# danielbrathwaite/OpenGL-Path-Tracing

Measured on AMD Instinct MI355X. Metric: Mrays/sec + ms/frame @1920×1080, 8 bounces, 1/2/4/8 MI355X, higher is better.
Workload: dtype f32; 1 GPU; C2: cornell 1920x1080, 1024 spp (frames 1..1024), 8 bounces (i<=8), AA+sky+sphere on; scene=cornell, width=1920, height=1080, spp=1024, max_bounce=8, frames_per_launch=1024, kernel_variant=0, parallelism=single GPU

## Files before the change

### opengl-path-tracing_amd/csrc/pt_cull.h

```cpp
#pragma once

#include "pt_math.h"

namespace ptc {

constexpr float kWindowLo = 0.0001f * 0x1.ff8p-1f;
constexpr float kWindowRay = 0x1.4p-20f;

PT_HD float min_t(float tf, float t) {
#if defined(__HIP_DEVICE_COMPILE__)
    return __builtin_amdgcn_fmed3f(tf, t, -__builtin_huge_valf());
#else
    return fminf(tf, t);
#endif
}

PT_HD void cull_addends(pt::f3 o, pt::f3 rd, const float cm[3], const float ws[3], pt::f3& ol, pt::f3& oh) {
    const pt::f3 ord = pt::mk(-(o.x * rd.x), -(o.y * rd.y), -(o.z * rd.z));
    const float ax = __builtin_fabsf(rd.x), ay = __builtin_fabsf(rd.y), az = __builtin_fabsf(rd.z);
    const pt::f3 e = pt::mk(__builtin_fmaf(cm[0], ax, 0x1p-17f * __builtin_fabsf(ord.x)),
                            __builtin_fmaf(cm[1], ay, 0x1p-17f * __builtin_fabsf(ord.y)),
                            __builtin_fmaf(cm[2], az, 0x1p-17f * __builtin_fabsf(ord.z)));
    const float omax = fmaxf(fmaxf(__builtin_fabsf(o.x), __builtin_fabsf(o.y)), __builtin_fabsf(o.z));
    const float wx = __builtin_fmaf(kWindowRay, omax, ws[0]), wy = __builtin_fmaf(kWindowRay, omax, ws[1]),
                wz = __builtin_fmaf(kWindowRay, omax, ws[2]);
    ol = ord - e;
    oh = ord + pt::mk(__builtin_fmaf(wx, ax, e.x), __builtin_fmaf(wy, ay, e.y), __builtin_fmaf(wz, az, e.z));
}

PT_HD bool cull_hit(float nx, float fx, float ny, float fy, float nz, float fz, pt::f3 rd, pt::f3 ol, pt::f3 oh,
                    float cur_t, float c_lo) {
    const float xn = __builtin_fmaf(nx, rd.x, ol.x), xf = __builtin_fmaf(fx, rd.x, oh.x);
    const float yn = __builtin_fmaf(ny, rd.y, ol.y), yf = __builtin_fmaf(fy, rd.y, oh.y);
    const float zn = __builtin_fmaf(nz, rd.z, ol.z), zf = __builtin_fmaf(fz, rd.z, oh.z);
    const float tn = fmaxf(fmaxf(xn, yn), zn);
    const float tf = fminf(fminf(xf, yf), zf);
    return fmaxf(tn, c_lo) <= min_t(tf, cur_t);
}

inline bool window_slack(const float* bvh, int n_nodes, const float* tris, float ws[3]) {
    const double u = 0x1p-24;
    const float inf = __builtin_huge_valf();
    ws[0] = ws[1] = ws[2] = 0.0f;
    if (n_nodes <= 0) return true;
    double M2 = 0.0;
    for (int q = 0; q < 3; q++) {
        const double m = fmax(fabs((double)bvh[q]), fabs((double)bvh[4 + q]));
        M2 += m * m;
    }
    M2 = sqrt(M2);
    double worst[3] = {0.0, 0.0, 0.0};
    for (int i = 0; i < n_nodes; i++) {
        const float* nd = bvh + 12 * (size_t)i;
        if (!(nd[8] > -1.0f)) continue;
        for (int k = 0; k < 2; k++) {
            const float* t = tris + 16 * (size_t)(int)nd[8 + k];
            const pt::f3 v0 = pt::mk(t[0], t[1], t[2]), v1 = pt::mk(t[4], t[5], t[6]), v2 = pt::mk(t[8], t[9], t[10]);
            const pt::f3 n = pt::normalize(pt::cross(v1 - v0, v2 - v0));
            const float d0 = -pt::dot(n, v0);
            if (!(fabs((double)n.x) + fabs((double)n.y) + fabs((double)n.z) < (double)inf)) continue;
            const double V[3][3] = {{v0.x, v0.y, v0.z}, {v1.x, v1.y, v1.z}, {v2.x, v2.y, v2.z}};
            const double nn[3] = {n.x, n.y, n.z};
            double E1[3], E2[3], L2 = 0.0, rho = 0.0;
            for (int q = 0; q < 3; q++) { E1[q] = V[1][q] - V[0][q]; E2[q] = V[2][q] - V[0][q]; }
            const double N[3] = {E1[1] * E2[2] - E2[1] * E1[2], E1[2] * E2[0] - E2[2] * E1[0], E1[0] * E2[1] - E2[0] * E1[1]};
            const double D = nn[0] * N[0] + nn[1] * N[1] + nn[2] * N[2];
            for (int a = 0; a < 3; a++) {
                const int b = (a + 1) % 3;
                double l2 = 0.0;
                for (int q = 0; q < 3; q++) l2 += (V[b][q] - V[a][q]) * (V[b][q] - V[a][q]);
                L2 = fmax(L2, l2);
                rho = fmax(rho, fabs(nn[0] * V[a][0] + nn[1] * V[a][1] + nn[2] * V[a][2] + (double)d0));
            }
            const double L = sqrt(L2);
            if (!(D > 0.0) || !(L2 <= 0x1p14 * D) || !(rho <= L)) return false;
            const double kappa = L2 / D, z = 1.06 * 0x1p-140 * L / D;
            const double sigma_t = u * (7.2 * M2 + 4.4 * fabs((double)d0)) + 1.14 * rho + 6.5 * z;
            for (int q = 0; q < 3; q++) {
                const double ext = fmax(fmax(V[0][q], V[1][q]), V[2][q]) - fmin(fmin(V[0][q], V[1][q]), V[2][q]);
                worst[q] = fmax(worst[q], 21.4 * u * kappa * ext + 1.021 * sigma_t + 2.0 * z);
            }
        }
    }
    for (int q = 0; q < 3; q++)
        if (!(worst[q] < 0x1p60)) return false;
    for (int q = 0; q < 3; q++) ws[q] = nextafterf((float)(1.25 * worst[q] * (1.0 + 0x1p-20)), inf);
    return true;
}

struct SweepRay { pt::f3 rp, rn, ol, oh; };
PT_HD SweepRay sweep_ray(pt::f3 rd, pt::f3 ol, pt::f3 oh) {
    SweepRay r;
    r.rp = pt::mk(rd.x > 0.0f ? rd.x : 0.0f, rd.y > 0.0f ? rd.y : 0.0f, rd.z > 0.0f ? rd.z : 0.0f);
    r.rn = pt::mk(rd.x > 0.0f ? 0.0f : rd.x, rd.y > 0.0f ? 0.0f : rd.y, rd.z > 0.0f ? 0.0f : rd.z);
    r.ol = ol;
    r.oh = oh;
    return r;
}
PT_HD bool sweep_hit(float lx, float hx, float ly, float hy, float lz, float hz, const SweepRay& r, float t0, float c_lo) {
    const float xn = __builtin_fmaf(lx, r.rp.x, __builtin_fmaf(hx, r.rn.x, r.ol.x));
    const float xf = __builtin_fmaf(hx, r.rp.x, __builtin_fmaf(lx, r.rn.x, r.oh.x));
    const float yn = __builtin_fmaf(ly, r.rp.y, __builtin_fmaf(hy, r.rn.y, r.ol.y));
    const float yf = __builtin_fmaf(hy, r.rp.y, __builtin_fmaf(ly, r.rn.y, r.oh.y));
    const float zn = __builtin_fmaf(lz, r.rp.z, __builtin_fmaf(hz, r.rn.z, r.ol.z));
    const float zf = __builtin_fmaf(hz, r.rp.z, __builtin_fmaf(lz, r.rn.z, r.oh.z));
    const float tn = fmaxf(fmaxf(xn, yn), zn);
    const float tf = fminf(fminf(xf, yf), zf);
    return fmaxf(tn, c_lo) <= min_t(tf, t0);
}
PT_HD unsigned sweep_push(unsigned m, bool hit) {
#if defined(__HIP_DEVICE_COMPILE__) && !defined(PT_SWEEP_NO_ADDC)
    unsigned r;
    const unsigned long long c = __builtin_amdgcn_ballot_w64(hit);
    unsigned long long co;
    asm("v_addc_co_u32 %0, %1, %2, %2, %3" : "=v"(r), "=s"(co) : "v"(m), "s"(c));
    return r;
#else
    return m + m + (hit ? 1u : 0u);
#endif
}
template <class T>
PT_HD unsigned sweep_mask(const SweepRay& r, float t0, float c_lo, T table, int n) {
    unsigned m = 0u;
    for (int k = n - 1; k >= 0; k--) {
        const auto a = table[2 * k], b = table[2 * k + 1];
        m = sweep_push(m, sweep_hit(a.x, a.y, a.z, a.w, b.x, b.y, r, t0, c_lo));
    }
    return m;
}
template <class T>
PT_HD unsigned sweep_mask(pt::f3 rd, pt::f3 ol, pt::f3 oh, float t0, float c_lo, T table, int n) {
    return sweep_mask(sweep_ray(rd, ol, oh), t0, c_lo, table, n);
}
PT_HD bool sweep_root_hit(const float box[6], const SweepRay& r, float t0, float c_lo) {
    return sweep_hit(box[0], box[1], box[2], box[3], box[4], box[5], r, t0, c_lo);
}

}
```

### opengl-path-tracing_amd/csrc/pt_render_phase.h

```cpp
namespace {

typedef float v4f __attribute__((ext_vector_type(4)));
typedef __attribute__((address_space(3))) const v4f lds_v4f;
typedef __attribute__((address_space(4))) const v4f const_v4f;

template <bool LDS>
__device__ __forceinline__ float4 tri_quad(const SceneView& S, int slot, int k) {
#ifdef PT_DIAG_TRIS_GLOBAL
    return S.tris[4 * slot + k];
#else
    return LDS ? S.tris[slot + k * S.tp] : S.tris[4 * slot + k];
#endif
}

using pt::in_guard;
using pt::in_range_abs;

using pt::win_open;
using pt::win_closed;

__device__ __forceinline__ int rank_in(unsigned long long m) {
    return (int)__builtin_amdgcn_mbcnt_hi((unsigned)(m >> 32), __builtin_amdgcn_mbcnt_lo((unsigned)m, 0u));
}

template <bool COMMON, bool SWEEP = false>
struct LaunchFacts {
    const KParams& p;
    __device__ __forceinline__ bool sweep() const { return COMMON ? SWEEP : p.sweep != 0; }
    __device__ __forceinline__ int mode() const { return COMMON ? 1 : p.mode; }
    __device__ __forceinline__ int flags() const { return COMMON ? 0 : p.flags; }
    __device__ __forceinline__ bool cons_walk() const { return COMMON || p.cons_walk != 0; }
    __device__ __forceinline__ bool scene_fast() const { return COMMON || p.scene_fast != 0; }
    __device__ __forceinline__ float win_lo() const { return COMMON ? ptc::kWindowLo : p.win_lo; }
    __device__ __forceinline__ int n_spheres() const { return COMMON ? 1 : p.sc.n_spheres; }
    __device__ __forceinline__ int tile_shift() const { return COMMON ? 0 : p.tile_shift; }
    __device__ __forceinline__ bool tile_perm() const { return COMMON || p.tile_perm != nullptr; }
    __device__ __forceinline__ bool tile_cost() const { return COMMON || p.tile_cost != nullptr; }
    __device__ __forceinline__ bool inside(int cx, int cy) const { return COMMON || ((cx < p.x_limit) & (cy < p.y_limit)); }
};

__device__ __forceinline__ void stage_tris_chain_order(float4* dst, const KParams& p, int T, int nthreads) {
    for (int i = threadIdx.x; i < 4 * T; i += nthreads) {
        const int slot = i >> 2, c = __float_as_int(p.sweep_tab[2 * (slot >> 1) + 1].w);
        dst[(i & 3) * T + 2 * c + (slot & 1)] = p.sc.tris[i];
    }
}

template <bool LDS, class Facts>
__device__ __forceinline__ bool shade_segment(const Facts& F, const KParams& p, const SceneView& S, bool hit, int hprim,
                                              float t, f3& o, f3& d, f3& inc, f3& col, uint32_t& state, int& bounce,
                                              f3& rgb) {
    bool finished = false;
    rgb = inc;
    if (hit && pt::length_gt_001(col)) {
        const f3 hitp = o + d * t;
        f3 normal;
        int mat;
        if (hprim >= 0) {
            const float4 nq = tri_quad<LDS>(S, hprim, 0);
            normal = mk(nq.x, nq.y, nq.z);
            mat = __float_as_int(tri_quad<LDS>(S, hprim, 2).w);
        } else {
            const int si = -2 - hprim;
            float4 s0 = S.spheres[2 * si];
            normal = pt::normalize(hitp - mk(s0.x, s0.y, s0.z));
            mat = __float_as_int(S.spheres[2 * si + 1].x);
        }
        if (pt::dot(normal, d) > 0.0f) normal = normal * -1.0f;
        if (F.mode() == 2) {
            rgb = (normal + mk(1, 1, 1)) * 0.5f;
            finished = true;
        } else if (F.mode() == 4) {
            float s = pt::length(hitp - o);
            float dist = 1.0f - pt::fsqrt(s + 1.0f) / (s + 1.0f);
            float q = dist * dist;
            rgb = mk(q, q, q);
            finished = true;
        } else {
            o = hitp;
            f3 diffuse = pt::normalize(normal + pt::random_unit_vector(state));
            float kk = 2.0f * pt::dot(normal, d);
            f3 specular = pt::normalize(d - normal * kk);
            float4 m0 = S.mats[3 * mat], m1 = S.mats[3 * mat + 1], m2 = S.mats[3 * mat + 2];
            if (F.mode() == 3) {
                rgb = mk(m0.x, m0.y, m0.z);
                finished = true;
            } else {
                float is_spec = (m1.w > pt::random01(state)) ? 1.0f : 0.0f;
                d = pt::mix(diffuse, specular, m0.w * is_spec);
                inc = inc + mk(m1.x, m1.y, m1.z) * col;
                col = col * pt::mix(mk(m0.x, m0.y, m0.z), mk(m2.x, m2.y, m2.z), is_spec);
                bounce++;
                if (bounce > p.max_bounce) {
                    rgb = inc;
                    finished = true;
                }
            }
        }
    } else {
        f3 env = mk(0, 0, 0);
        if (!(F.flags() & PT_FLAG_NO_SKY)) {
            f3 dir = pt::normalize(d);
            float tt = 0.5f * (dir.z + 1.0f);
            float omt = 1.0f - tt;
            env = mk(omt * 1.0f + tt * 0.5f, omt * 1.0f + tt * 0.7f, omt * 1.0f + tt * 1.0f);
        }
        rgb = inc + env * col;
        finished = true;
    }
    return finished;
}

struct QueueIds { unsigned id, qnext, qend; };
template <bool SPLIT>
__device__ __forceinline__ QueueIds queue_ids(const KParams& p, bool want, unsigned long long m, unsigned qnext,
                                              unsigned qend) {
    const unsigned need = (unsigned)__popcll(m);
    const unsigned rank = (unsigned)rank_in(m);
    const int leader = __ffsll((long long)m) - 1;
    unsigned id;
    if (SPLIT && qend - qnext >= need) {
        id = qnext + rank;
        qnext += need;
    } else {
        const unsigned avail = SPLIT ? qend - qnext : 0u;
        const unsigned take = SPLIT ? max(need - avail, (unsigned)p.pull_batch) : need;
        unsigned base = 0;
        if (want && rank == 0u) base = atomicAdd(p.work_counter, take);
        base = (unsigned)__builtin_amdgcn_readlane((int)base, leader);
        id = rank < avail ? qnext + rank : base + (rank - avail);
        if (SPLIT) {
            qnext = base + (need - avail);
            qend = base + take;
        }
    }
    const QueueIds q = {id, qnext, qend};
    return q;
}

template <class Facts>
__device__ __forceinline__ void camera_ray(const Facts& F, const KParams& p, f3 cpos, f3 cfwd, f3 cright, f3 cup, int lx,
                                           int y, int k, int r, uint32_t& state, f3& o, f3& d, f3& inc, f3& col,
                                           int& bounce) {
    if (r == 0) state = pt::seed(lx, y, p.frame_first + k);
    float ax = 0.0f, ay = 0.0f;
    if (!(F.flags() & PT_FLAG_NO_AA)) {
        ax = pt::random01(state);
        ay = pt::random01(state);
    }
    float u = pt::div_mk((float)lx + ax, p.fW, p.rW) - 0.5f;
    float v = pt::div_mk((float)y + ay, p.fH, p.rH) - 0.5f;
    d = pt::normalize((cfwd + cright * u) + cup * v);
    o = cpos;
    inc = mk(0, 0, 0);
    col = mk(1, 1, 1);
    bounce = 0;
}

template <class Facts>
__device__ __forceinline__ bool seg_in_guard(const Facts& F, f3 o, f3 d) {
    return F.scene_fast() & in_guard(o.x, 0x1p-40f, 0x1p60f) & in_guard(o.y, 0x1p-40f, 0x1p60f) &
           in_guard(o.z, 0x1p-40f, 0x1p60f) & in_range_abs(d.x, 0x1p-20f, 2.0f) &
           in_range_abs(d.y, 0x1p-20f, 2.0f) & in_range_abs(d.z, 0x1p-20f, 2.0f);
}

__device__ __forceinline__ float sphere_t(const SceneView& S, int si, f3 o, f3 d) {
    float4 s0 = S.spheres[2 * si];
    f3 oc = o - mk(s0.x, s0.y, s0.z);
    float a = pt::dot(d, d);
    float half_b = pt::dot(oc, d);
    float cq = pt::dot(oc, oc) - s0.w;
    float disc = half_b * half_b - a * cq;
    return disc < 0.0f ? -1.0f : (-half_b - pt::sqrt_g(disc)) / a;
}

__device__ __forceinline__ unsigned sweep_candidates(const KParams& p, const SceneView& S, const const_v4f* sweep_tab,
                                                     bool on, f3 o, f3 rd, float t) {
    unsigned cand = 0u;
    if (on) {
        f3 ol, oh;
        ptc::cull_addends(o, rd, S.cm, S.ws, ol, oh);
        const ptc::SweepRay sr = ptc::sweep_ray(rd, ol, oh);
        bool in = true;
        if (p.sweep_root) in = ptc::sweep_root_hit(p.root_box, sr, t, S.clo);
        if (in) cand = ptc::sweep_mask(sr, t, S.clo, sweep_tab, p.n_sweep);
    }
    return cand;
}

struct LeafChoice { bool c1, c2; };
__device__ __forceinline__ LeafChoice leaf_choice(float h1, float h2, float t) {
    const bool c1 = win_open(h1, t) & ((h1 < h2) | (h2 < 0.0001f));
    const bool c2 = !c1 & win_open(h2, t);
    const LeafChoice r = {c1, c2};
    return r;
}

}
```

### opengl-path-tracing_amd/csrc/pt_render_pool.h

```cpp
namespace {

__device__ __forceinline__ void pool_cold_walk(const KParams& p, const SceneView& S, f3 o, f3 d, float& t, int& hprim) {
    int w = 0;
    while (w >= 0) {
        const float4 lo = p.sc.nodes[2 * w], hi = p.sc.nodes[2 * w + 1];
        const int a = __float_as_int(hi.z), b = __float_as_int(hi.w);
        if (!slab(lo, hi, o, d, t)) { w = b; continue; }
        if (a >= 0) { w = a; continue; }
        const int q = (~a) >> 2;
        const int s0 = 2 * __float_as_int(p.sweep_tab[2 * q + 1].w);
        const bool cop = __float_as_int(tri_quad<true>(S, s0 + 1, 1).w) != 0;
        const float4 nda = tri_quad<true>(S, s0, 0);
        const float4 ndb = cop ? nda : tri_quad<true>(S, s0 + 1, 0);
        const float ta = tri_plane(nda, o, d);
        const float tb = cop ? ta : tri_plane(ndb, o, d);
        bool oka = false, okb = false, ca = false, cb = false;
        if (win_open(ta, t)) oka = tri_edges_at<true, false>(S, s0, mk(nda.x, nda.y, nda.z), o + d * ta, false, 0.0f, ca);
        if (win_closed(tb, t)) okb = tri_edges_at<true, false>(S, s0 + 1, mk(ndb.x, ndb.y, ndb.z), o + d * tb, false, 0.0f, cb);
        const float h1 = oka ? ta : -1.0f, h2 = okb ? tb : -1.0f;
        const LeafChoice lc = leaf_choice(h1, h2, t);
        if (lc.c1 | lc.c2) {
            t = lc.c1 ? h1 : h2;
            hprim = s0 + (lc.c1 ? 0 : 1);
        }
        w = b;
    }
}

__device__ __forceinline__ void pool_pass_fence() {
    __builtin_amdgcn_fence(__ATOMIC_RELEASE, "wavefront");
    __builtin_amdgcn_wave_barrier();
    __builtin_amdgcn_fence(__ATOMIC_ACQUIRE, "wavefront");
}

template <int NT, int P, int MINW>
__global__ __launch_bounds__(NT, MINW) void k_render_pool(KParams p) {
    static_assert(P >= 64 && P <= ptpool::kMaxPaths && P % 4 == 0, "one-byte list entries in a 16-byte padded array");
    using namespace ptpool;
    const LaunchFacts<true, true> F{p};
    const const_v4f* const sweep_tab = (const const_v4f*)(size_t)p.sweep_tab;
    resolve_frames(p);
    extern __shared__ float4 lds[];
    const int T = p.n_slots, nt = 4 * T, nm = 3 * p.n_mats, ns = 2, nb = 2 * p.n_sweep;
    stage_tris_chain_order(lds, p, T, NT);
    for (int i = threadIdx.x; i < nm; i += NT) lds[nt + i] = p.sc.mats[i];
    for (int i = threadIdx.x; i < ns; i += NT) lds[nt + nm + i] = p.sc.spheres[i];
    for (int i = threadIdx.x; i < nb; i += NT) lds[nt + nm + ns + i] = p.sweep_tab[i];
    const int scene_q = nt + nm + ns + nb;
    const int lane = (int)(threadIdx.x & 63u);
    float4* const pool = lds + scene_q + (int)(threadIdx.x >> 6) * (wave_bytes(P) / 16);
    unsigned char* const list = (unsigned char*)(pool + kChunks * P);
    for (int i = lane; i < P; i += kLanes) {
        pool[quad_of(kChunkO, i, P)] = make_float4(0, 0, 0, -1.0f);
        pool[quad_of(kChunkD, i, P)] = make_float4(0, 0, 1, 0);
        pool[quad_of(kChunkInc, i, P)] = make_float4(0, 0, 0, __uint_as_float(pack_hit(-1, -1)));
        pool[quad_of(kChunkCol, i, P)] = make_float4(1, 1, 1, 0);
        pool[quad_of(kChunkItem, i, P)] = make_float4(__uint_as_float(kNoItem), 0, 0, 0);
        list[i] = (unsigned char)i;
    }
    __syncthreads();
    SceneView S;
    S.nodes = nullptr;
    S.tris = lds;
    S.mats = lds + nt;
    S.spheres = lds + nt + nm;
    const float4* const boxes = lds + nt + nm + ns;
    S.np = 0;
    S.tp = T;
    S.cm[0] = p.cons_m[0], S.cm[1] = p.cons_m[1], S.cm[2] = p.cons_m[2];
    S.ws[0] = p.win_slack[0], S.ws[1] = p.win_slack[1], S.ws[2] = p.win_slack[2];
    S.clo = ptc::kWindowLo;
    const f3 cpos = mk(p.cam[0], p.cam[1], p.cam[2]), cfwd = mk(p.cam[3], p.cam[4], p.cam[5]);
    const f3 cright = mk(p.cam[6], p.cam[7], p.cam[8]), cup = mk(p.cam[9], p.cam[10], p.cam[11]);
    const int tiles_x = (p.W + 7) >> 3;
    const unsigned n_groups = (unsigned)((p.n_frames + p.group - 1) / p.group);
    const unsigned total_ids = p.queue_tiles * n_groups * 64u;
    unsigned qnext = 0, qend = 0;
    Lists L = {P, 0};
    while (L.nS + L.nL > 0) {
        const int phase = choose(L), n = take(L, phase);
        const bool on = lane < n;
        int idx = 0;
        if (on) idx = list[pop_index(L, phase, n, lane, P)];
        drop(L, phase, n);
        bool to_shade = false, to_leaf = false;
        if (phase == kShade) {
            const float4 c0 = pool[quad_of(kChunkO, idx, P)], c1 = pool[quad_of(kChunkD, idx, P)];
            const float4 c2 = pool[quad_of(kChunkInc, idx, P)], c3 = pool[quad_of(kChunkCol, idx, P)];
            const float4 c4 = pool[quad_of(kChunkItem, idx, P)];
            f3 o = mk(c0.x, c0.y, c0.z), d = mk(c1.x, c1.y, c1.z), inc = mk(c2.x, c2.y, c2.z), col = mk(c3.x, c3.y, c3.z);
            float t = c0.w;
            unsigned bi = __float_as_uint(c1.w);
            int hprim = hit_hprim(__float_as_uint(c2.w)), bounce = hit_bounce(__float_as_uint(c2.w));
            uint32_t state = __float_as_uint(c3.w);
            unsigned xy = __float_as_uint(c4.x);
            int aidx = __float_as_int(c4.y);
            int k = k_k(__float_as_uint(c4.z)), kend = k_kend(__float_as_uint(c4.z));
            unsigned pcost = cost_of(__float_as_uint(c4.w));
            bool report = cost_report(__float_as_uint(c4.w));
            bool retired = false;
            if (on && !(t < 0.0f)) {
                const bool hit = hprim != -1;
                pcost++;
                f3 rgb;
                const bool finished = shade_segment<true>(F, p, S, hit, hprim, t, o, d, inc, col, state, bounce, rgb);
                if (finished) {
                    bounce = -1;
                    const f3 px = (mk(0, 0, 0) + rgb) / 1.0f;
                    nt_store3(p.rgb + 3 * ((size_t)k * (size_t)(p.rows_local * p.W) + (size_t)aidx), px);
                    k++;
                }
                t = -1.0f;
            }
            if (on & (bounce < 0) & (xy != kNoItem) & (k >= kend)) {
                if (report) atomicAdd(&p.tile_cost[(xy_crow(xy) >> 3) * tiles_x + (xy_lx(xy) >> 3)], pcost);
                xy = kNoItem;
            }
            const bool want = on && xy == kNoItem;
            const unsigned long long m = __ballot(want);
            if (m) {
                const QueueIds qi = queue_ids<true>(p, want, m, qnext, qend);
                const unsigned id = qi.id;
                qnext = qi.qnext, qend = qi.qend;
                if (want) {
                    if (id >= total_ids) {
                        retired = true;
                    } else {
                        const unsigned item = id >> 6, w = id & 63u;
                        const unsigned tile = p.grp_magic ? __umulhi(item, p.grp_magic) : item;
                        const int g = (int)(item - tile * n_groups);
                        const unsigned pk = p.tile_perm[tile];
                        const int tx = (int)(pk & 0xffffu), ty = (int)(pk >> 16);
                        const int cx = tx * 8 + (int)(w & 7u);
                        const int crow = ty * 8 + (int)(w >> 3);
                        if ((cx < p.W) & (crow < p.rows_local)) {
                            xy = pack_xy(cx, crow);
                            aidx = crow * p.W + cx;
                            report = (w & 0x1bu) == 0u;
                            pcost = 0;
                            k = g * p.group;
                            kend = min(k + p.group, p.n_frames);
                            bounce = -1;
                        }
                    }
                }
            }
            if (on && xy != kNoItem) {
                const int lx = xy_lx(xy), y = p.row0 + xy_crow(xy) * p.row_stride;
                if (bounce < 0) camera_ray(F, p, cpos, cfwd, cright, cup, lx, y, k, 0, state, o, d, inc, col, bounce);
                const bool fast_seg = seg_in_guard(F, o, d);
                const f3 rd = fast_seg ? mk(pt::rcp_fast(d.x), pt::rcp_fast(d.y), pt::rcp_fast(d.z)) : mk(0, 0, 0);
                t = __builtin_huge_valf();
                hprim = -1;
                {
                    const float ht = sphere_t(S, 0, o, d);
                    if (win_open(ht, t)) {
                        t = ht;
                        hprim = -2;
                    }
                }
                const bool walk = !ray_has_nan(o, d);
                const unsigned cand = sweep_candidates(p, S, sweep_tab, walk & fast_seg, o, rd, t);
                const bool cold = walk & !fast_seg;
                if (__any(cold)) {
                    if (cold) pool_cold_walk(p, S, o, d, t, hprim);
                }
                bi = cand;
                to_leaf = cand != 0u;
            }
            to_shade = on & !retired & !to_leaf;
            if (on) {
                pool[quad_of(kChunkO, idx, P)] = make_float4(o.x, o.y, o.z, t);
                pool[quad_of(kChunkD, idx, P)] = make_float4(d.x, d.y, d.z, __uint_as_float(bi));
                pool[quad_of(kChunkInc, idx, P)] = make_float4(inc.x, inc.y, inc.z, __uint_as_float(pack_hit(hprim, bounce)));
                pool[quad_of(kChunkCol, idx, P)] = make_float4(col.x, col.y, col.z, __uint_as_float(state));
                pool[quad_of(kChunkItem, idx, P)] = make_float4(__uint_as_float(xy), __int_as_float(aidx),
                                                                __uint_as_float(pack_k(k, kend)),
                                                                __uint_as_float(pack_cost(pcost, report)));
            }
        } else {
            const float4 c0 = pool[quad_of(kChunkO, idx, P)], c1 = pool[quad_of(kChunkD, idx, P)];
            float* const hw = (float*)&pool[quad_of(kChunkInc, idx, P)] + 3;
            const unsigned hb = __float_as_uint(*hw);
            const f3 o = mk(c0.x, c0.y, c0.z), d = mk(c1.x, c1.y, c1.z);
            float t = c0.w;
            unsigned bi = __float_as_uint(c1.w);
            const bool at = on;
            int s0 = 0, lp = 0;
            bool cop = false;
            float4 nd0 = make_float4(0, 0, 0, 0);
            if (at) {
                lp = __ffs((int)bi) - 1;
                s0 = 2 * lp;
                cop = __float_as_int(tri_quad<true>(S, s0 + 1, 1).w) != 0;
                nd0 = tri_quad<true>(S, s0, 0);
            }
            float h1 = -1.0f, h2 = -1.0f;
            bool ca = false, cb = false;
            leaf_pair_tests<true, false>(S, at, s0, nd0, cop, o, d, t, p.compact_max, h1, h2, false, ca, cb);
            bool c1h = false, c2h = false;
            if (at) {
                const LeafChoice lc = leaf_choice(h1, h2, t);
                c1h = lc.c1, c2h = lc.c2;
            }
            const bool chk = at & (c1h | c2h);
            if (__any(chk)) {
                if (chk) {
                    const f3 rd = mk(pt::rcp_fast(d.x), pt::rcp_fast(d.y), pt::rcp_fast(d.z));
                    if (!slab_fast(boxes[2 * lp], boxes[2 * lp + 1], o, d, rd, t)) c1h = c2h = false;
                }
            }
            if (at) {
                int hprim = hit_hprim(hb);
                if (c1h | c2h) {
                    t = c1h ? h1 : h2;
                    hprim = s0 + (c1h ? 0 : 1);
                }
                bi &= bi - 1u;
                to_leaf = bi != 0u;
                to_shade = bi == 0u;
                ((float*)&pool[quad_of(kChunkO, idx, P)])[3] = t;
                ((float*)&pool[quad_of(kChunkD, idx, P)])[3] = __uint_as_float(bi);
                *hw = __uint_as_float(with_hprim(hb, hprim));
            }
        }
        const unsigned long long mS = __ballot(to_shade), mL = __ballot(to_leaf);
        if (to_shade) list[push_index(L, kShade, rank_in(mS), P)] = (unsigned char)idx;
        if (to_leaf) list[push_index(L, kLeaf, rank_in(mL), P)] = (unsigned char)idx;
        grow(L, kShade, __popcll(mS));
        grow(L, kLeaf, __popcll(mL));
        pool_pass_fence();
    }
}

}
```

Measured before the change: 35190 Mrays/s.

## Software-pipeline sweep box tests with double-buffered chunk loads from LDS

```diff
diff --git a/opengl-path-tracing_amd/csrc/pt_cull.h b/opengl-path-tracing_amd/csrc/pt_cull.h
--- a/opengl-path-tracing_amd/csrc/pt_cull.h
+++ b/opengl-path-tracing_amd/csrc/pt_cull.h
@@ -128,6 +128,59 @@
     }
     return m;
 }
+#if defined(__clang__)
+#define PT_SWEEP_UNROLL _Pragma("unroll")
+#else
+#define PT_SWEEP_UNROLL
+#endif
+PT_HD void sweep_issue_fence() {
+#if defined(__HIP_DEVICE_COMPILE__)
+    __builtin_amdgcn_sched_barrier(0);
+#endif
+}
+template <int D> struct SweepChunk { float q[D][6]; };
+template <int D, class T>
+PT_HD void sweep_chunk_load(SweepChunk<D>& c, T table, int k) {
+    PT_SWEEP_UNROLL
+    for (int j = 0; j < D; j++) {
+        const auto a = table[2 * (k - j)], b = table[2 * (k - j) + 1];
+        c.q[j][0] = a.x, c.q[j][1] = a.y, c.q[j][2] = a.z, c.q[j][3] = a.w, c.q[j][4] = b.x, c.q[j][5] = b.y;
+    }
+}
+template <int D>
+PT_HD unsigned sweep_chunk_test(unsigned m, const SweepChunk<D>& c, const SweepRay& r, float t0, float c_lo) {
+    PT_SWEEP_UNROLL
+    for (int j = 0; j < D; j++)
+        m = sweep_push(m, sweep_hit(c.q[j][0], c.q[j][1], c.q[j][2], c.q[j][3], c.q[j][4], c.q[j][5], r, t0, c_lo));
+    return m;
+}
+template <int D, class T>
+PT_HD unsigned sweep_mask_piped(const SweepRay& r, float t0, float c_lo, T table, int n) {
+    static_assert(D >= 1 && D <= 8, "boxes in flight");
+    unsigned m = 0u;
+    int k = n - 1;
+    for (int j = n % D; j > 0; j--, k--) {
+        const auto a = table[2 * k], b = table[2 * k + 1];
+        m = sweep_push(m, sweep_hit(a.x, a.y, a.z, a.w, b.x, b.y, r, t0, c_lo));
+    }
+    if (k < 0) return m;
+    SweepChunk<D> ca, cb;
+    sweep_chunk_load(ca, table, k);
+    for (; k >= 3 * D - 1; k -= 2 * D) {
+        sweep_chunk_load(cb, table, k - D);
+        sweep_issue_fence();
+        m = sweep_chunk_test(m, ca, r, t0, c_lo);
+        sweep_chunk_load(ca, table, k - 2 * D);
+        sweep_issue_fence();
+        m = sweep_chunk_test(m, cb, r, t0, c_lo);
+    }
+    if (k >= 2 * D - 1) {
+        sweep_chunk_load(cb, table, k - D);
+        m = sweep_chunk_test(m, ca, r, t0, c_lo);
+        return sweep_chunk_test(m, cb, r, t0, c_lo);
+    }
+    return sweep_chunk_test(m, ca, r, t0, c_lo);
+}
 template <class T>
 PT_HD unsigned sweep_mask(pt::f3 rd, pt::f3 ol, pt::f3 oh, float t0, float c_lo, T table, int n) {
     return sweep_mask(sweep_ray(rd, ol, oh), t0, c_lo, table, n);
diff --git a/opengl-path-tracing_amd/csrc/pt_render_phase.h b/opengl-path-tracing_amd/csrc/pt_render_phase.h
--- a/opengl-path-tracing_amd/csrc/pt_render_phase.h
+++ b/opengl-path-tracing_amd/csrc/pt_render_phase.h
@@ -174,7 +174,8 @@
     return disc < 0.0f ? -1.0f : (-half_b - pt::sqrt_g(disc)) / a;
 }
 
-__device__ __forceinline__ unsigned sweep_candidates(const KParams& p, const SceneView& S, const const_v4f* sweep_tab,
+template <int DEPTH = 0, class Table>
+__device__ __forceinline__ unsigned sweep_candidates(const KParams& p, const SceneView& S, Table table,
                                                      bool on, f3 o, f3 rd, float t) {
     unsigned cand = 0u;
     if (on) {
@@ -183,7 +184,8 @@
         const ptc::SweepRay sr = ptc::sweep_ray(rd, ol, oh);
         bool in = true;
         if (p.sweep_root) in = ptc::sweep_root_hit(p.root_box, sr, t, S.clo);
-        if (in) cand = ptc::sweep_mask(sr, t, S.clo, sweep_tab, p.n_sweep);
+        if (in) cand = DEPTH > 0 ? ptc::sweep_mask_piped<(DEPTH > 0 ? DEPTH : 1)>(sr, t, S.clo, table, p.n_sweep)
+                                 : ptc::sweep_mask(sr, t, S.clo, table, p.n_sweep);
     }
     return cand;
 }
diff --git a/opengl-path-tracing_amd/csrc/pt_render_pool.h b/opengl-path-tracing_amd/csrc/pt_render_pool.h
--- a/opengl-path-tracing_amd/csrc/pt_render_pool.h
+++ b/opengl-path-tracing_amd/csrc/pt_render_pool.h
@@ -1,3 +1,9 @@
+#ifndef PT_POOL_SWEEP_DEPTH
+#define PT_POOL_SWEEP_DEPTH 2
+#endif
+#ifndef PT_POOL_SWEEP_LDS
+#define PT_POOL_SWEEP_LDS 1
+#endif
 namespace {
 
 __device__ __forceinline__ void pool_cold_walk(const KParams& p, const SceneView& S, f3 o, f3 d, float& t, int& hprim) {
@@ -39,6 +45,7 @@
     using namespace ptpool;
     const LaunchFacts<true, true> F{p};
     const const_v4f* const sweep_tab = (const const_v4f*)(size_t)p.sweep_tab;
+    (void)sweep_tab;
     resolve_frames(p);
     extern __shared__ float4 lds[];
     const int T = p.n_slots, nt = 4 * T, nm = 3 * p.n_mats, ns = 2, nb = 2 * p.n_sweep;
@@ -160,7 +167,11 @@
                     }
                 }
                 const bool walk = !ray_has_nan(o, d);
-                const unsigned cand = sweep_candidates(p, S, sweep_tab, walk & fast_seg, o, rd, t);
+#if PT_POOL_SWEEP_DEPTH > 0 && PT_POOL_SWEEP_LDS
+                const unsigned cand = sweep_candidates<PT_POOL_SWEEP_DEPTH>(p, S, boxes, walk & fast_seg, o, rd, t);
+#else
+                const unsigned cand = sweep_candidates<PT_POOL_SWEEP_DEPTH>(p, S, sweep_tab, walk & fast_seg, o, rd, t);
+#endif
                 const bool cold = walk & !fast_seg;
                 if (__any(cold)) {
                     if (cold) pool_cold_walk(p, S, o, d, t, hprim);
```

New measurement: 37070 Mrays/s (median of 6 runs). +5.3%, better.
